# KLab/YAIK

Hardware: AMD Instinct MI355X
Metric: Mpix/s tile encode (alpha reject + 7 gradient passes + 8x8 range quant), 8K RGBA (higher is better)
Workload: dtype u8/int32 (+f32 mode-selection sums)

## Files before the change

### yaik_amd/csrc/yk_api.hip

```cpp
#include "yk_common.h"
#ifdef YK_TEST_HOOKS
#include "../../include/yaik_hip_test.h"
#endif
#include <cstdio>
#include <cstring>
#include <utility>
#include <vector>

int yk_fail(yk_ctx* c, int code, const char* what, hipError_t e) {
    if (c && c->err.empty()) {
        c->err = what ? what : "error";
        if (e != hipSuccess) { c->err += ": "; c->err += hipGetErrorString(e); }
    }
    return code;
}

int yk_refuse(yk_ctx* c, int code, const char* what) {
    if (c) c->err = what ? what : "error";
    return code;
}

static void yk_input_changed(yk_ctx* c) {
    c->encoded = false; c->alphaDone = false; c->alphaFinished = false; c->avBatchValid = false; c->mipValid = false; c->img.sb.valid = false; c->pal.valid = false;
    c->cornersReady = false; c->ppActive = false; c->ppLastBit = 0; c->previewFresh = false;
// ... 26 lines not shown
    YK_HIP(c, M.alphaUnitBox.alloc(s, yk_alpha_units(c->fullW, c->mtH) * F * 4, 16));
    static const int sh[7][2] = { {4,4},{4,3},{3,4},{3,3},{3,2},{2,3},{2,2} };
    size_t cur = 0, oBm[7], oBm0b, oCov, oInfo, oRun;
    auto place = [&](size_t bytesPerFrame) { const size_t o = cur; cur = up(cur + bytesPerFrame * F + 16, 256); return o; };
    for (int i = 0; i < 7; i++) {
        const int bx = (sh[i][0] == 2) ? 32 : 64, by = (sh[i][1] == 2) ? 32 : 64;
        const size_t bits = (size_t)((c->fullW + bx - 1) / bx) * ((c->h + by - 1) / by) * ((bx >> sh[i][0]) * (by >> sh[i][1]));
        c->bitmapBytes[i] = bits >> 3;
        fs.bitmap[i] = up(c->bitmapBytes[i] + 4, 16);
        oBm[i] = place(fs.bitmap[i]);
    }
    const size_t nB64 = (size_t)((c->fullW + 63) / 64) * ((c->h + 63) / 64);
    fs.bm0b = up(nB64 * 4, 16); oBm0b = place(fs.bm0b);
    fs.coverage = up(MT, 8); oCov = place(fs.coverage * sizeof(uint16_t));
    fs.tileInfo = up(T8, 2); oInfo = place(fs.tileInfo * sizeof(uint2));
    fs.runSums = up((T8 + 7) / 8, 4); oRun = place(fs.runSums * sizeof(uint32_t));
    if (cur >= ((size_t)1 << 32)) return yk_fail(c, YK_ERR_BAD_ARG, "image too large for 32-bit offsets into the small-output arena");
    YK_HIP(c, M.small.alloc(s, cur));
    YK_HIP(c, hipMemset(M.small, 0, cur));
    B.small = M.small;
    for (int i = 0; i < 7; i++) B.bitmap[i] = B.small + oBm[i];
    B.bm0b = B.small + oBm0b; B.coverage = reinterpret_cast<uint16_t*>(B.small + oCov);
    B.tileInfo = reinterpret_cast<uint2*>(B.small + oInfo); B.runSums = reinterpret_cast<uint32_t*>(B.small + oRun);
    fs.tileDef = 3 * T8; fs.tileCount = 3 * T8; fs.slots = 3 * T8 * YK_SLOT;
    YK_HIP(c, M.tileDef.alloc(s, fs.tileDef * F, 16));
    YK_HIP(c, M.tileCount.alloc(s, fs.tileCount * F, 16));
    YK_HIP(c, M.slots.alloc(s, fs.slots * F, 16));
    c->nScanBlocks = (int)((T8 + 1023) / 1024);
    fs.blockN = (size_t)c->nScanBlocks * 2;
    YK_HIP(c, M.blockSums.alloc(s, fs.blockN * F));
    YK_HIP(c, M.blockCnt.alloc(s, fs.blockN * F));
    YK_HIP(c, hipMemset(M.blockCnt, 0, fs.blockN * F * sizeof(uint32_t)));
    YK_HIP(c, M.totals.alloc(s, 8 * F));
    fs.defsOut = 3 * T8;
    YK_HIP(c, M.defsOut.alloc(s, fs.defsOut * F, 16));
    c->nibStride = T8 * YK_SLOT + 64;
    fs.nibOut = 3 * c->nibStride;
    YK_HIP(c, M.nibOut.alloc(s, fs.nibOut * F, 16));
    B.keep = M.keep; B.bounds = M.bounds; B.tileDef = M.tileDef; B.tileCount = M.tileCount; B.slots = M.slots;
    B.blockSums = M.blockSums; B.blockCnt = M.blockCnt; B.totals = M.totals; B.defsOut = M.defsOut; B.nibOut = M.nibOut;
    c->dstValid = false;
    return YK_OK;
}
static int yk_alloc_image(yk_ctx* c) {
    const int rc = yk_alloc_image_run(c);
    if (rc) yk_free_image(c);
// ... 759 lines not shown
```

### yaik_amd/csrc/yk_common.h

```cpp
#pragma once
#include <hip/hip_runtime.h>
#include <stdint.h>
#include <stddef.h>
#include <memory>
#include <string>
#include <vector>
#include "../../include/yaik_hip.h"

#define YK_BLK      64
#define YK_LSTRIDE  68
#define YK_LROWS    65
#define YK_EV_RING  64
#define YK_SLOT     32
#define YK_NUM_STAGES 11
#define YK_STAGE_RING 16

struct YkFrameStrides {
    unsigned long long plane, keep, bitmap[7], coverage, tileDef, tileCount, slots, blockN, defsOut, nibOut;
    unsigned long long bm0b, tileInfo, runSums;
};

enum { YK_EVSET_ALPHA = 1, YK_EVSET_PACK = 2 };
enum { YK_EV_A0, YK_EV_E0, YK_EV_E1, YK_EV_P1, YK_EV_N };
struct YkEvRing {
    hipEvent_t ev[YK_EV_RING][YK_EV_N] = {};
    YkEvRing() = default;
    YkEvRing(const YkEvRing&) = delete; YkEvRing& operator=(const YkEvRing&) = delete;
    ~YkEvRing() { for (auto& set : ev) for (hipEvent_t e : set) if (e) (void)hipEventDestroy(e); }
};

// ... 23 lines not shown
    int w, h;
    int hAvail;
    int y0;
    int fullH;
    int rejectFactor, startMode, wantDst;
    int ablate;
    const uint8_t* keep;
    const int32_t* bounds;
    uint8_t* bitmap[7];
    uint16_t* coverage;
    uint16_t* tileDef;
    uint8_t*  tileCount;
    uint8_t*  slots;
    uint32_t* blockCnt;
    int32_t*  dst[3];
    int tilesW, tilesH, mtW, mtH;
    int xBB64, yBB64, xBB32, yBB32;
    int nFrames;
    const uint8_t* qtab;
    uint8_t* small;
    uint32_t oBm[7], oBm0b, oCov, oInfo, oRun;
    uint4* pixCache;
    YkFrameStrides fs;
};

#define YK_SB_COUNTS 9
struct YkStreamRec { uint8_t* rgb[7]; uint8_t* pix; uint8_t* type; };
struct YkStreamsBatch {
    YkBuf<uint32_t> owner;
    YkBuf<uint32_t> cScratch;
    YkBuf<uint32_t> r1Scratch;
    YkBuf<uint32_t> counts;
    YkBuf<uint8_t> out;
    YkBuf<YkStreamRec> tab;
    std::vector<yk_frame_streams> table; bool valid = false;
    int what = 0;
};

struct YkPalette {
    YkBuf<uint8_t> scratch;
    YkBuf<uint8_t> out;
    YkBuf<uint32_t> carry;
    bool carryFresh = true;
    std::vector<uint8_t> segHost;
    std::vector<uint32_t> lenBase;
    int nSeg = 0; bool valid = false;
};

struct YkPaletteDec {
    YkBuf<uint8_t> scratch;
    YkBuf<uint8_t> out;
    YkBuf<uint8_t> stage;
    std::vector<size_t> slotOff, slotLen;
    std::vector<uint32_t> statusHost;
    size_t statusOff = 0;
    int nSeg = 0; bool valid = false;
};

#ifndef YK_ALPHA_R
#define YK_ALPHA_R 4
#endif
static inline size_t yk_alpha_units(int fullW, int mtH) { return (size_t)((fullW / 4 + 63) / 64) * (size_t)((mtH + YK_ALPHA_R - 1) / YK_ALPHA_R); }

struct YkImageBufs {
    YkBuf<uint8_t> keep; YkBuf<int32_t> bounds;
    YkBuf<int> alphaUnitBox;
    YkBuf<uint8_t> small;
    YkBuf<uint16_t> tileDef; YkBuf<uint8_t> tileCount, slots;
    YkBuf<int32_t> dst[3];
    YkBuf<uint32_t> blockSums, blockCnt, totals;
    YkBuf<unsigned long long> exportSizes;
    YkBuf<uint16_t> defsOut; YkBuf<uint8_t> nibOut;
    YkBuf<uint32_t> latticeOwner; YkBuf<uint8_t> cornerStream; YkBuf<uint32_t> cornerScratch;
    YkBuf<uint32_t> cornerEdgeIdx;
    YkBuf<uint16_t> covCh;
    YkBuf<uint8_t> mapped3;
    YkBuf<uint32_t> ppBitmap; YkBuf<uint8_t> ppStream; YkBuf<uint32_t> ppScratch;
    YkBuf<int32_t> preview;
    YkBuf<uint8_t> r1Slots, r1Params; YkBuf<uint32_t> r1Cnt; YkBuf<uint8_t> r1Pix, r1Type;
    YkBuf<uint4> pixCache;
    YkStreamsBatch sb;
};

struct yk_ctx {
    int device = -1;
    int numCU = 256;
    const uint8_t* qtab = nullptr;
    hipStream_t ownStream = nullptr;
    hipStream_t stream = nullptr;
    std::string err;
    int fullW = 0, fullH = 0, nPlanes = 0, y0 = 0, h = 0, halo = 0;
    int tilesW = 0, tilesH = 0, mtW = 0, mtH = 0;
    int nFrames = 1, curFrame = 0;
    YkFrameStrides fs = {};
    struct Bases {
        const int32_t* plane[4];
        uint8_t* keep;
        int32_t* bounds;
        uint8_t* bitmap[7]; uint16_t* coverage; uint16_t* tileDef; uint8_t* tileCount; uint8_t* slots;
        uint32_t* blockSums;
        uint32_t* blockCnt;
        uint32_t* totals;
        uint16_t* defsOut;
        uint8_t* nibOut;
        uint8_t* small;
        uint8_t* bm0b; uint2* tileInfo; uint32_t* runSums;
    } B = {};
    int strideElems = 0;
    YkBuf<int32_t> ownedPlanes;
    YkBuf<uint8_t> pxStage;
    hipEvent_t evPixCopy = nullptr;
    int boundsOff = 8;
    bool alphaDone = false, alphaFinished = false;
    int32_t hostBounds[4] = {0, 0, 0, 0}; int hostDiscard = 1, hostHasChunk = 0;
    size_t bitmapBytes[7] = {};
    int32_t dstFill = -1; bool dstValid = false;
    hipEvent_t evHandoff = nullptr;
// ... 128 lines not shown
```

### yaik_amd/csrc/yk_encode2.hip

```cpp
#include "yk_common.h"
#include "yk_curves.h"
#include "yk_device.h"
#include <mutex>

__constant__ float c_curve2[6][16] = YK_CURVE_TABLE;

#define LS YK_LSTRIDE
#ifdef YK_TEST_HOOKS
#define YK2_ABLATE(bit) ((P.ablate & (bit)) != 0)
#else
#define YK2_ABLATE(bit) false
#endif

__device__ __forceinline__ int y2_byte(uint32_t w, int ch) { return (w >> (8 * ch)) & 255; }
__device__ __forceinline__ uint32_t y2_absdiff(uint32_t a, uint32_t b) { uint32_t r; asm("v_sad_u32 %0, %1, %2, 0" : "=v"(r) : "v"(a), "v"(b)); return r; }
__device__ __forceinline__ int y2_round6(int v) { return (v & ~3) | (v >> 6); }
__device__ __forceinline__ int y2_round6p(int v) { v = min(v + 1, 255); return (v & ~3) | (v >> 6); }

typedef short y2s2 __attribute__((ext_vector_type(2)));
typedef unsigned short y2u2 __attribute__((ext_vector_type(2)));
__device__ __forceinline__ y2u2 y2_u2(uint32_t w) { return __builtin_bit_cast(y2u2, w); }
__device__ __forceinline__ y2s2 y2_s2(y2u2 v) { return __builtin_bit_cast(y2s2, v); }
__device__ __forceinline__ y2u2 y2_splat(int v) { const unsigned short t = (unsigned short)v; return (y2u2){ t, t }; }
__device__ __forceinline__ y2s2 y2_splats(int v) { const short t = (short)v; return (y2s2){ t, t }; }
// ... 454 lines not shown
        int L[16];
        for (int i = 0; i < cnt; i++) {
            L[i] = __float2int_rz(__fadd_rn((float)BN, __fmul_rn(c_curve2[m][i], (float)R)));
            if (L[i] != BN + __float2int_rz(__fmul_rn(c_curve2[m][i], (float)R))) bad++;
        }
        for (int v = mn; v <= mx; v++) {
            int best = 1 << 30, bi = 0;
            for (int n = 0; n < cnt; n++) { const int dd = abs(L[n] - v); if (dd < best) { best = dd; bi = n; } }
            const uint4 row = tab[(size_t)(R - YK2_QR0) * YK2_QROWS + (v - BN + 2)];
            const uint32_t w = m < 2 ? row.x : (m < 4 ? row.y : row.z);
            const uint32_t hb = (m & 1) ? (w >> 16) : (w & 0xFFFFu);
            const int ix = (row.w >> (4 * m)) & 15;
            if (hb != y2_f16_bits(best) || ix != bi) bad++;
        }
    }
    if (bad) atomicAdd(mismatches, bad);
}

#define YK2_RUN 16
template <int K> __device__ __forceinline__ uint32_t y2_writelane_k(uint32_t v, uint32_t old) { asm("v_writelane_b32 %0, %1, %2" : "+v"(old) : "s"(v), "n"(K)); return old; }
__device__ __forceinline__ uint32_t y2_writelane(uint32_t v, int k, uint32_t old) {
    switch (k) {
        case 0: return y2_writelane_k<0>(v, old); case 1: return y2_writelane_k<1>(v, old); case 2: return y2_writelane_k<2>(v, old);
        case 3: return y2_writelane_k<3>(v, old); case 4: return y2_writelane_k<4>(v, old); default: return y2_writelane_k<5>(v, old);
    }
}
#ifdef YK2_TIMING
__device__ unsigned long long g_y2_times[65536 * 16];
#define YK2_PROBE(i) do { if ((i) == 0 && lane == 0 && unit < 65536) { g_y2_times[(size_t)unit * 16 + 10] = 0; g_y2_times[(size_t)unit * 16 + 11] = 0; g_y2_times[(size_t)unit * 16 + 12] = y2_t_entry; g_y2_times[(size_t)unit * 16 + 13] = ((unsigned long long)y2_xcc << 32) | y2_hwid; } if (lane == 0 && unit < 65536) { g_y2_times[(size_t)unit * 16 + 2 * (i)] = __builtin_amdgcn_s_memtime(); g_y2_times[(size_t)unit * 16 + 2 * (i) + 1] = __builtin_amdgcn_s_memrealtime(); } } while (0)
extern "C" int yk_debug_wave_times(unsigned long long* out) { return (int)hipMemcpyFromSymbol(out, HIP_SYMBOL(g_y2_times), sizeof(g_y2_times)); }
#else
#define YK2_PROBE(i) do { } while (0)
#endif
#define YK2_LUTW 84
#ifndef YK2_WIN
#define YK2_WIN 16
#endif
#ifndef YK2_PREF
#define YK2_PREF 8
#endif
#ifndef YK2_RVWIN
#define YK2_RVWIN 8
#endif

#define Y2_QUAD_X 0xB1
#define Y2_QUAD_Y 0x4E
template <int CTRL> __device__ __forceinline__ int y2_quad(int v) { return __builtin_amdgcn_update_dpp(v, v, CTRL, 0xF, 0xF, true); }
// ... 30 lines not shown
}

template <bool WANT_DST, bool MODE3>
__global__ __launch_bounds__(64, 4) void yk_encode2_kernel(const YkEncodeParams P) {
    constexpr int kStart = MODE3 ? 3 : 0;
    constexpr int kPixWords = 17 * LS, kLutWords = WANT_DST ? 16 * YK2_LUTW : 0;
    __shared__ __attribute__((aligned(16))) uint32_t s_mem[kPixWords > kLutWords ? kPixWords : kLutWords];
    uint32_t* const s_pix = s_mem;
    uint32_t (*const s_lut)[YK2_LUTW] = reinterpret_cast<uint32_t (*)[YK2_LUTW]>(s_mem);
    __shared__ uint32_t s_bm[24];
    __shared__ uint8_t s_list[64];
    __shared__ __attribute__((aligned(16))) float s_curve[WANT_DST ? 6 : 1][16];
    __shared__ __attribute__((aligned(16))) float s_rcp[256];
    __shared__ __attribute__((aligned(16))) uint32_t s_aux[432];
    uint32_t* const s_lat = s_aux;
    float (*const s_chain)[68] = reinterpret_cast<float (*)[68]>(s_aux);
    float* const s_err = reinterpret_cast<float*>(s_aux + 408);
    __shared__ uint32_t s_range[3 * 64];
    __shared__ __attribute__((aligned(16))) uint32_t s_sp[3 * 4 * 8 + 3 * 4 * 16];

    uint32_t* const s_tile = s_aux + 416;
    __shared__ uint32_t s_iwTest[WANT_DST ? 1024 : 1];
    uint32_t* const s_iw = WANT_DST ? s_iwTest : s_mem;
    static_assert(WANT_DST || kPixWords >= 1024, "index words need 4 KB");

    const int lane = threadIdx.x;
    __builtin_amdgcn_s_setprio(3);
#ifdef YK2_TIMING
    const unsigned long long y2_t_entry = __builtin_amdgcn_s_memrealtime();
    const unsigned y2_hwid = __builtin_amdgcn_s_getreg((4 << 0) | (0 << 6) | (31 << 11)), y2_xcc = __builtin_amdgcn_s_getreg((20 << 0) | (0 << 6) | (31 << 11));
#endif
    typedef const __attribute__((address_space(4))) YkEncodeParams* Y2ParamPtr;
    auto strip = [&](const int slot, const int xcd, const int lane, Y2ParamPtr const Pp) {
    const __attribute__((address_space(4))) YkEncodeParams& P = *Pp;
    const int nBf = P.xBB64 * P.yBB64, nB = nBf * P.nFrames;
    const int grp = slot / (YK2_RUN * 4);
    const int unit = (grp * 8 + ((xcd + grp) & 7)) * (YK2_RUN * 4) + (slot - grp * (YK2_RUN * 4));
    int L = unit >> 2; const int wave = unit & 3;
    if (L >= nB) return;
    size_t fr = 0;
    if (P.nFrames > 1) { fr = (size_t)(L / nBf); L -= (int)fr * nBf; }
    const int32_t* const pl0 = P.plane[0] + fr * P.fs.plane; const int32_t* const pl1 = P.plane[1] + fr * P.fs.plane; const int32_t* const pl2 = P.plane[2] + fr * P.fs.plane;
    const uint8_t* const keepP = P.keep ? P.keep + fr * P.fs.keep : nullptr;
    const int32_t* const boundsP = P.bounds ? P.bounds + fr * 16 : nullptr;
    uint8_t* const slotsP = P.slots + fr * P.fs.slots;
    uint32_t* const blockCntP = P.blockCnt + fr * P.fs.blockN;
    const int BY = L / P.xBB64, BX = L - BY * P.xBB64;
    const int w = P.w, h = P.h;

    YK2_PROBE(0);
    if (lane < 24) s_bm[lane] = 0;
    {
        const int g4 = (lane & 15) * 4, r0 = lane >> 4;
        const int gx = BX * 64 + g4;
        const bool inX = gx + 3 < w;
        const int gxc = min(gx, w - 4);
        const int gyS = BY * 64 + wave * 16;
        const int gyB = min(gyS, P.hAvail - 1);
        const size_t rowBase = (size_t)gyB * (size_t)P.strideElems;
        const char* const b0 = reinterpret_cast<const char*>(pl0 + rowBase);
        const char* const b1 = reinterpret_cast<const char*>(pl1 + rowBase);
        const char* const b2 = reinterpret_cast<const char*>(pl2 + rowBase);
        int4 R[4], G[4], B[4];
#pragma unroll
        for (int k = 0; k < 4; k++) {
            const int rel = min(gyS + r0 + 4 * k, P.hAvail - 1) - gyB;
            const uint32_t off = (uint32_t)(rel * P.strideElems + gxc) * 4u;
            R[k] = *reinterpret_cast<const int4*>(b0 + off);
            G[k] = *reinterpret_cast<const int4*>(b1 + off);
            B[k] = *reinterpret_cast<const int4*>(b2 + off);
        }
        int4 Rb, Gb, Bb;
        {
            const int rel = min(gyS + 16, P.hAvail - 1) - gyB;
            const uint32_t off = (uint32_t)(rel * P.strideElems + gxc) * 4u;
            Rb = *reinterpret_cast<const int4*>(b0 + off);
            Gb = *reinterpret_cast<const int4*>(b1 + off);
            Bb = *reinterpret_cast<const int4*>(b2 + off);
        }
        uint32_t hcol;
        const int hr = min(max(lane - 32, 0), 16);
        {
            const int rel = min(gyS + hr, P.hAvail - 1) - gyB;
            const uint32_t off = (uint32_t)(rel * P.strideElems + min(BX * 64 + 64, w - 1)) * 4u;
            hcol = y2_pack3(*reinterpret_cast<const int32_t*>(b0 + off), *reinterpret_cast<const int32_t*>(b1 + off), *reinterpret_cast<const int32_t*>(b2 + off));
        }
        const float4 rc4 = *reinterpret_cast<const float4*>(P.qtab + YK2_QBYTES + (size_t)lane * 16);

        __builtin_amdgcn_s_setprio(0);
        uint4 o[4], ob;
#pragma unroll
        for (int k = 0; k < 4; k++) {
            o[k] = make_uint4(y2_pack3(R[k].x, G[k].x, B[k].x), y2_pack3(R[k].y, G[k].y, B[k].y), y2_pack3(R[k].z, G[k].z, B[k].z), y2_pack3(R[k].w, G[k].w, B[k].w));
            *reinterpret_cast<uint4*>(&s_pix[(r0 + 4 * k) * LS + g4]) = o[k];
        }
        ob = make_uint4(y2_pack3(Rb.x, Gb.x, Bb.x), y2_pack3(Rb.y, Gb.y, Bb.y), y2_pack3(Rb.z, Gb.z, Bb.z), y2_pack3(Rb.w, Gb.w, Bb.w));
        if (lane < 16) *reinterpret_cast<uint4*>(&s_pix[16 * LS + g4]) = ob;
        if (BX * 64 + 64 > w) {
            if (!inX) {
#pragma unroll
                for (int k = 0; k < 4; k++) *reinterpret_cast<uint4*>(&s_pix[(r0 + 4 * k) * LS + g4]) = make_uint4(o[k].w, o[k].w, o[k].w, o[k].w);
                if (lane < 16) *reinterpret_cast<uint4*>(&s_pix[16 * LS + g4]) = make_uint4(ob.w, ob.w, ob.w, ob.w);
            }
        }
        if (lane >= 32 && lane <= 48) s_pix[hr * LS + 64] = hcol;
        *reinterpret_cast<float4*>(&s_rcp[lane * 4]) = rc4;

    }
    __syncthreads();
    YK2_PROBE(1);

    const int q = lane >> 4, cx = y2_cell_x(lane & 15), cy = y2_cell_y(lane & 15);
    const int bxCell = q * 16 + cx * 4, byCell = wave * 16 + cy * 4;
    const int gxCell = BX * 64 + bxCell, gyCell = BY * 64 + byCell;
    const int lcell = (cy * 4) * LS + bxCell;
    const int lat = cy * 17 + q * 4 + cx;
    const bool mtIn = (BX * 64 + q * 16 < w) && (BY * 64 + wave * 16 < h);

    uint32_t pw[16];
#pragma unroll
    for (int r = 0; r < 4; r++) {
        const uint4 t = *reinterpret_cast<const uint4*>(&s_pix[lcell + r * LS]);
        pw[r * 4 + 0] = t.x; pw[r * 4 + 1] = t.y; pw[r * 4 + 2] = t.z; pw[r * 4 + 3] = t.w;
    }

    unsigned long long cov = 0ULL;
    unsigned long long evaluated = 0ULL;
    {
        bool dead = !mtIn;
        {
            const int lim = 4 * P.rejectFactor + 1;
// ... 28 lines not shown
            y2s2 rg[16], bb[8];
#pragma unroll
            for (int k = 0; k < 16; k++) rg[k] = y2_rg(pw[k]);
#pragma unroll
            for (int k = 0; k < 8; k++) bb[k] = y2_bb(pw[2 * k], pw[2 * k + 1]);
            const Y2Pass S = { s_lat, lat, cx, cy, rg, bb, deadLanes, stripInside, gxCell, gyCell, w, h, P.rejectFactor, s_bm, bxCell, byCell, s_pix, s_list, s_range, lane };
            if (deadLanes == 0ULL) y2_grad_pass<4, 4, true>(S, cov, evaluated);
            else y2_grad_pass<4, 4>(S, cov, evaluated);
            if (~(cov | deadLanes) != 0ULL) {
                y2_grad_pass<4, 3>(S, cov, evaluated);
                y2_grad_pass<3, 4>(S, cov, evaluated);
                y2_grad_pass<3, 3>(S, cov, evaluated);
                y2_grad_pass<3, 2>(S, cov, evaluated);
                y2_grad_pass<2, 3>(S, cov, evaluated);
                y2_grad_pass<2, 2>(S, cov, evaluated);
            }
#pragma unroll
            for (int r = 0; r < 4; r++) {
                const uint4 t = *reinterpret_cast<const uint4*>(&s_pix[lcell + r * LS]);
                pw[r * 4 + 0] = t.x; pw[r * 4 + 1] = t.y; pw[r * 4 + 2] = t.z; pw[r * 4 + 3] = t.w;
            }
        }
    }
    const int mtIdx = ((BY * 64 + wave * 16) >> 4) * P.mtW + ((BX * 64 + q * 16) >> 4);
    __syncthreads();
    YK2_PROBE(2);
    uint8_t* const small = P.small;
    const uint32_t bmv = s_bm[lane < 24 ? lane : 0];
    auto bmWord = [&](const int k) -> uint32_t { return (uint32_t)__builtin_amdgcn_readlane((int)bmv, k); };
    const uint32_t i64 = (uint32_t)(BY * P.xBB64 + BX);
    const uint32_t frU = (uint32_t)fr;
    uint32_t off32 = ~0u, val32 = 0u;
    {
        const uint32_t w1 = (uint32_t)wave & 1u, w2 = (uint32_t)wave >> 1;
        uint32_t off8 = 0u, val8 = 0u;
        off8 = y2_writelane(P.oBm0b + frU * (uint32_t)P.fs.bm0b + i64 * 4u + (uint32_t)wave, 0, off8);
        val8 = y2_writelane((bmWord(0) >> (4 * wave)) & 0xFu, 0, val8);
        off8 = y2_writelane(P.oBm[1] + frU * (uint32_t)P.fs.bitmap[1] + i64 * 4u + (uint32_t)wave, 1, off8);
        val8 = y2_writelane(bmWord(1) >> (8 * wave), 1, val8);
        off8 = y2_writelane(P.oBm[2] + frU * (uint32_t)P.fs.bitmap[2] + i64 * 4u + (uint32_t)wave, 2, off8);
        val8 = y2_writelane(bmWord(2) >> (8 * wave), 2, val8);
        if (lane < 3) *(small + off8) = (uint8_t)val8;
        const unsigned long long t = ((cov >> 2) ^ cov) & 0x0C0C0C0C0C0C0C0CULL;
        const unsigned long long covRM = cov ^ t ^ (t << 2);
        uint32_t off16 = ((lane & 15) == 0 && mtIn) ? P.oCov + (frU * (uint32_t)P.fs.coverage + (uint32_t)mtIdx) * 2u : ~0u;
        uint32_t val16 = (uint32_t)((covRM >> (q * 16)) & 0xFFFFULL);
        off16 = y2_writelane(P.oBm[3] + frU * (uint32_t)P.fs.bitmap[3] + (i64 * 4u + (uint32_t)wave) * 2u, 1, off16);
        val16 = y2_writelane(bmWord(3 + (int)w2) >> (16 * w1), 1, val16);
#pragma unroll
        for (int sx = 0; sx < 2; sx++) {
            const bool in = BX * 2 + sx < P.xBB32;
            off16 = y2_writelane(in ? P.oBm[5] + frU * (uint32_t)P.fs.bitmap[5] + ((uint32_t)((BY * P.xBB32 + BX * 2 + sx) * 4 + wave)) * 2u : ~0u, 2 + sx, off16);
            val16 = y2_writelane(bmWord(9 + sx * 2 + (int)w2) >> (16 * w1), 2 + sx, val16);
        }
        if (off16 != ~0u) *reinterpret_cast<uint16_t*>(small + off16) = (uint16_t)val16;
        if (P.pixCache != nullptr) {
            const bool cellIn = (gxCell < w) && (gyCell < h);
            if (cellIn && !((cov >> lane) & 1ULL)) {
                const uint32_t strip = (uint32_t)((BY * 4 + wave) * P.xBB64 + BX);
                uint4* dstp = P.pixCache + (size_t)strip * 256 + lane;
#pragma unroll
                for (int r = 0; r < 4; r++) dstp[r * 64] = make_uint4(pw[r * 4 + 0], pw[r * 4 + 1], pw[r * 4 + 2], pw[r * 4 + 3]);
            }
        }
        {
            const bool in = BY * 2 + (int)w2 < P.yBB32;
            off32 = y2_writelane(in ? P.oBm[4] + frU * (uint32_t)P.fs.bitmap[4] + ((uint32_t)(((BY * 2 + (int)w2) * P.xBB64 + BX) * 2) + w1) * 4u : ~0u, 1, off32);
            val32 = y2_writelane(bmWord(5 + (int)w2 * 2 + (int)w1), 1, val32);
#pragma unroll
            for (int sx = 0; sx < 2; sx++) {
                const bool in6 = in && (BX * 2 + sx < P.xBB32);
                off32 = y2_writelane(in6 ? P.oBm[6] + frU * (uint32_t)P.fs.bitmap[6] + ((uint32_t)(((BY * 2 + (int)w2) * P.xBB32 + BX * 2 + sx) * 2) + w1) * 4u : ~0u, 2 + sx, off32);
                val32 = y2_writelane(bmWord(13 + ((int)w2 * 2 + sx) * 2 + (int)w1), 2 + sx, val32);
            }
        }
    }
    YK2_PROBE(3);
    int cxB = 0, cyB = 0, cw = w, chh = P.fullH, discard = 1;
    if (boundsP) {
        const int b0 = boundsP[0], b1 = boundsP[1], b2 = boundsP[2], b3 = boundsP[3];
        discard = (b0 == 0 && b1 == 0 && b2 == w && b3 == P.fullH) ? 1 : 0;
        cxB = (b0 >> 3) << 3; cyB = (b1 >> 3) << 3;
        cw = (((b2 + 7) >> 3) << 3) - cxB; chh = (((b3 + 7) >> 3) << 3) - cyB;
    }
    const int cxl = cx & 1, cyl = cy & 1;
    const int tgx = gxCell - cxl * 4, tgyl = gyCell - cyl * 4, tgy = tgyl + P.y0;
    const bool tileIn = (tgx + 8 <= w) && (tgyl + 8 <= h);
    const bool part = tileIn && tgx >= cxB && tgx < cxB + cw && tgy >= cyB && tgy < cyB + chh && (tgx + 8 <= cw) && (tgy + 8 <= chh);
    const bool keepMT = (keepP == nullptr) || discard || (mtIn && keepP[mtIdx] != 0);
    const bool tileLive = part && keepMT;
    const int l00 = lane & ~3;
    const uint32_t quadN = (uint32_t)((~cov) >> l00) & 15u;
    const int v00 = (int)(quadN & 1u), v01 = (int)((quadN >> 2) & 1u);
    const bool valid = tileLive && ((quadN >> (lane & 3)) & 1u);
    const int nTop = __popc(quadN & 3u), nBot = __popc(quadN >> 2);
    const int tileIdx = (tgyl >> 3) * P.tilesW + (tgx >> 3);
    const size_t T8 = (size_t)P.tilesW * P.tilesH;
    const int tw = lane >> 2;
    const bool writer = ((lane & 3) == 0) && tileIn;
    const unsigned long long validMask = __ballot(valid);
    const bool fullTiles = !WANT_DST && __ballot(tileLive && quadN != 15u && quadN != 0u) == 0ULL;

    {
        const int n16 = (tileLive && !YK2_ABLATE(1)) ? (nTop + nBot) : 0;
        if ((P.tilesW & 7) == 0) {
#pragma unroll
            for (int r = 0; r < 2; r++) {
                const bool mine = writer && ((cy >> 1) == r);
                const unsigned long long b0 = __ballot(mine && (n16 & 1)), b1 = __ballot(mine && (n16 & 2)), b2 = __ballot(mine && (n16 & 4));
                const unsigned long long bd = __ballot(mine && n16 > 0);
                const int row = ((BY * 64 + wave * 16) >> 3) + r;
                off32 = y2_writelane(row < P.tilesH ? P.oRun + (frU * (uint32_t)P.fs.runSums + (uint32_t)(row * (P.tilesW >> 3) + BX)) * 4u : ~0u, 4 + r, off32);
                val32 = y2_writelane((uint32_t)(__popcll(b0) + 2 * __popcll(b1) + 4 * __popcll(b2)) | ((uint32_t)__popcll(bd) << 16), 4 + r, val32);
            }
        } else if (writer && n16 > 0) {
            atomicAdd(&blockCntP[((size_t)tileIdx >> 10) * 2], 16u * (uint32_t)n16);
            atomicAdd(&blockCntP[((size_t)tileIdx >> 10) * 2 + 1], 1u);
        }
        if (off32 != ~0u) *reinterpret_cast<uint32_t*>(small + off32) = val32;
    }

    YK2_STAT(70, validMask != 0ULL ? 1 : 0); YK2_STAT(74, __popcll(validMask));
    { const int nv = __popcll(validMask); YK2_STAT(120 + (nv == 0 ? 0 : nv <= 4 ? 1 : nv <= 8 ? 2 : nv <= 16 ? 3 : nv <= 32 ? 4 : nv < 64 ? 5 : 6), 1); (void)nv; }
    uint32_t defs01 = 0u, defs2c = 0u;
    if (validMask != 0ULL && !YK2_ABLATE(1)) {
        uint32_t* lut = &s_lut[WANT_DST ? tw : 0][0];
        if (WANT_DST) {
            s_curve[lane >> 4][lane & 15] = c_curve2[lane >> 4][lane & 15];
            if (lane < 32) s_curve[4 + (lane >> 4)][lane & 15] = c_curve2[4 + (lane >> 4)][lane & 15];
        }
        const int j4 = lane & 3;
        const int nValidLanes = __popcll(validMask);
        const bool spread = nValidLanes <= 4 && !WANT_DST;
        const int vRank = (int)__builtin_amdgcn_mbcnt_hi((uint32_t)(validMask >> 32), __builtin_amdgcn_mbcnt_lo((uint32_t)validMask, 0u));
        uint32_t slotOff[4];
#pragma unroll
        for (int r = 0; r < 4; r++) {
            const int yIn = cyl * 4 + r;
            const int pos = (yIn < 4) ? (yIn * 4 * nTop + (cxl ? 4 * v00 : 0))
                                      : (16 * nTop + (yIn - 4) * 4 * nBot + (cxl ? 4 * v01 : 0));
            slotOff[r] = (uint32_t)tileIdx * (uint32_t)YK_SLOT + (uint32_t)(pos >> 1);
        }
        int tmn[3], tmx[3];
        {
            y2u2 mnRB = y2_splat(0xFFFF), mxRB = y2_splat(0), mnG = y2_splat(0xFFFF), mxG = y2_splat(0);
            if (valid) {
#pragma unroll
                for (int k = 0; k < 16; k += 2) {
// ... 331 lines not shown
        hipLaunchKernelGGL(yk_qtab_kernel, dim3(YK2_QNR), dim3(320), 0, c->stream, reinterpret_cast<uint4*>(t));
        {
            float rcp[256]; rcp[0] = 0.0f;
            for (int v = 1; v < 256; v++) rcp[v] = 1.0f / (float)v;
            YK_HIP(c, hipMemcpyAsync(t + YK2_QBYTES, rcp, sizeof rcp, hipMemcpyHostToDevice, c->stream));
        }
        hipLaunchKernelGGL(yk_deftab_kernel, dim3(225), dim3(YK2_DEFN1), 0, c->stream, reinterpret_cast<uint32_t*>(t + YK2_QBYTES + YK2_RCPBYTES));
        YK_HIP(c, hipGetLastError());
        YK_HIP(c, hipStreamSynchronize(c->stream));
        g_qtab[c->device] = t;
    }
    c->qtab = g_qtab[c->device];
    return YK_OK;
}
void yk_selftest_qtab_launch(yk_ctx* c, int* mismatches) {
    hipLaunchKernelGGL(yk_selftest_qtab_kernel, dim3(256), dim3(256), 0, c->stream, reinterpret_cast<const uint4*>(c->qtab),
                       reinterpret_cast<const uint32_t*>(c->qtab + YK2_QBYTES + YK2_RCPBYTES), mismatches);
}

int yk_launch_encode2(yk_ctx* c, const YkEncodeParams& P) {
    if (!P.qtab) return yk_fail(c, YK_ERR_STATE, "quantiser table missing");
    if (P.startMode != 0 && P.startMode != 3) return yk_fail(c, YK_ERR_BAD_ARG, "startMode must be 0 or 3");
    const int nB = P.xBB64 * P.yBB64 * P.nFrames, group = 8 * YK2_RUN;
    dim3 grid(((nB + group - 1) / group) * group * 4);
    if (P.wantDst) {
        if (P.startMode) hipLaunchKernelGGL((yk_encode2_kernel<true, true>), grid, dim3(64), 0, c->stream, P);
        else hipLaunchKernelGGL((yk_encode2_kernel<true, false>), grid, dim3(64), 0, c->stream, P);
    } else {
        if (P.startMode) hipLaunchKernelGGL((yk_encode2_kernel<false, true>), grid, dim3(64), 0, c->stream, P);
        else hipLaunchKernelGGL((yk_encode2_kernel<false, false>), grid, dim3(64), 0, c->stream, P);
    }
    YK_HIP(c, hipGetLastError());
    return YK_OK;
}
```

### yaik_amd/csrc/yk_stages.hip

```cpp
#include "yk_common.h"
#ifdef YK_TEST_HOOKS
#include "../../include/yaik_hip_test.h"
#endif
#include "yk_device.h"

typedef int yk_i4 __attribute__((ext_vector_type(4)));
#ifndef YK_ALPHA_WAVES
#define YK_ALPHA_WAVES 3
#endif
__global__ __launch_bounds__(64 * YK_ALPHA_WAVES, 4) void yk_alpha_kernel(const int32_t* __restrict__ alpha0, int strideElems, int w, int h, int y0,
                                                      uint8_t* __restrict__ keep0, int mtW, int mtH, unsigned long long planeStride,
                                                      unsigned long long keepStride, yk_i4* __restrict__ unitBox0, unsigned total) {
    const int lane = threadIdx.x & 63;
    const int vecPerRow = w >> 2;
    const int nSeg = (vecPerRow + 63) >> 6;
    const int nUnits = nSeg * ((mtH + YK_ALPHA_R - 1) / YK_ALPHA_R);
    const unsigned uu = blockIdx.x * YK_ALPHA_WAVES + (threadIdx.x >> 6);
    if (uu >= total) return;
    const int f = (int)(uu / (unsigned)nUnits), u = (int)(uu - (unsigned)f * (unsigned)nUnits);
    const int32_t* alpha = alpha0 + (size_t)f * planeStride;
    uint8_t* keep = keep0 + (size_t)f * keepStride;
    const int tyU = u / nSeg, seg = u - tyU * nSeg, ty0 = tyU * YK_ALPHA_R;
    const int xv = seg * 64 + lane;
    const bool inX = xv < vecPerRow;
// ... 269 lines not shown
    return YK_OK;
}

int yk_launch_encode(yk_ctx* c, int rejectFactor, int mode3BitOnly, int wantDst, bool batch) {
    const YkFrameView V = yk_frame(c, batch ? 0 : c->curFrame);
    YkEncodeParams P;
    for (int i = 0; i < 4; i++) P.plane[i] = V.plane[i];
    P.strideElems = c->strideElems; P.w = c->fullW; P.h = c->h; P.hAvail = c->h + c->halo; P.y0 = c->y0; P.fullH = c->fullH;
    P.rejectFactor = rejectFactor; P.startMode = mode3BitOnly ? 3 : 0; P.wantDst = wantDst; P.ablate = c->ablate;
    P.keep = (c->nPlanes == 4) ? V.keep : nullptr;
    P.bounds = (c->nPlanes == 4) ? V.bounds + c->boundsOff : nullptr;
    for (int i = 0; i < 7; i++) P.bitmap[i] = V.bitmap[i];
    P.coverage = V.coverage; P.tileDef = V.tileDef; P.tileCount = V.tileCount; P.slots = V.slots;
    P.blockCnt = c->kernelVersion == 2 ? V.blockCnt : nullptr;
    for (int i = 0; i < 3; i++) P.dst[i] = c->img.dst[i];
    P.tilesW = c->tilesW; P.tilesH = c->tilesH; P.mtW = c->mtW; P.mtH = c->mtH;
    P.xBB64 = (c->fullW + 63) / 64; P.yBB64 = (c->h + 63) / 64; P.xBB32 = (c->fullW + 31) / 32; P.yBB32 = (c->h + 31) / 32;
    P.nFrames = batch ? c->nFrames : 1; P.fs = c->fs;
    P.qtab = c->qtab;
    P.small = V.small;
    auto off = [&](const void* p) { return (uint32_t)(static_cast<const uint8_t*>(p) - V.small); };
    for (int i = 0; i < 7; i++) P.oBm[i] = off(V.bitmap[i]);
    P.oBm0b = off(V.bm0b); P.oCov = off(V.coverage); P.oInfo = off(V.tileInfo); P.oRun = off(V.runSums);
    P.pixCache = nullptr; c->pixCacheValid = false;
    if (c->pixCacheOn && !batch && c->kernelVersion == 2 && c->nFrames == 1) {
        if (!c->img.pixCache) YK_HIP(c, c->img.pixCache.alloc(c->stream, (size_t)P.xBB64 * 64 * ((size_t)(c->h + 15) / 16 * 16) / 4, 4096));
        P.pixCache = c->img.pixCache; c->pixCacheValid = true;
    }
    if (c->kernelVersion == 2) return yk_launch_encode2(c, P);
    if (batch) return yk_fail(c, YK_ERR_STATE, "batches need kernel version 2");
    if (c->nPlanes == 4) {
        hipLaunchKernelGGL(yk_alpha_publish_kernel, dim3(1), dim3(1), 0, c->stream, V.bounds, c->boundsOff, c->fullW, c->fullH);
        P.bounds = V.bounds;
    }
    if (!g_crossCheckLauncher) return yk_fail(c, YK_ERR_STATE, "kernel version 1 is not part of this library: register it with yk_set_cross_check_launcher");
    if (g_crossCheckLauncher(c->stream, &P) != 0) return yk_fail(c, YK_ERR_HIP, "cross-check kernel launch", hipGetLastError());
    return YK_OK;
}

int yk_launch_pack(yk_ctx* c, bool batch) {
    const size_t T8 = (size_t)c->tilesW * c->tilesH;
    const int nb = c->nScanBlocks, F = batch ? c->nFrames : 1;
    const YkFrameView V = yk_frame(c, batch ? 0 : c->curFrame);
    if (c->kernelVersion != 2) hipLaunchKernelGGL(yk_scan1_kernel, dim3(nb), dim3(1024), 0, c->stream, V.tileCount, T8, V.blockCnt);
    const bool v2 = c->kernelVersion == 2;
    const uint32_t* runSums = (v2 && (c->tilesW & 7) == 0) ? V.runSums : nullptr;
// ... 78 lines not shown
```

Measured before the change: 235,800.

## Table-drive bitmap output offsets, hoist keep/bounds scalar loads, use magic division

Precomputes a per-wave, per-lane output geometry table on the host so the kernel's small-arena bitmap and run-sum writes become a single table lookup, replacing chains of writelane and address arithmetic. Keep and bounds are fetched early with scalar loads that overlap with the pixel loads. Integer divisions by the block width and frame size become multiply-shift magic division. Spare waves no longer exit before the early loads, and a host verification tool for the divider is added. This adds a table allocation and a limit on block count per launch, and relies on inline asm and on the table staying in sync with the layout.

```diff
diff --git a/yaik_amd/csrc/yk_api.hip b/yaik_amd/csrc/yk_api.hip
--- a/yaik_amd/csrc/yk_api.hip
+++ b/yaik_amd/csrc/yk_api.hip
@@ -72,6 +72,17 @@
     for (int i = 0; i < 7; i++) B.bitmap[i] = B.small + oBm[i];
     B.bm0b = B.small + oBm0b; B.coverage = reinterpret_cast<uint16_t*>(B.small + oCov);
     B.tileInfo = reinterpret_cast<uint2*>(B.small + oInfo); B.runSums = reinterpret_cast<uint32_t*>(B.small + oRun);
+    {
+        YkOutGeom g;
+        for (int i = 0; i < 7; i++) g.oBm[i] = (uint32_t)oBm[i];
+        g.oBm0b = (uint32_t)oBm0b; g.oRun = (uint32_t)oRun;
+        g.xBB64 = (c->fullW + 63) / 64; g.xBB32 = (c->fullW + 31) / 32; g.yBB32 = (c->h + 31) / 32; g.tilesW = c->tilesW; g.tilesH = c->tilesH;
+        YkOutRow tab[4][YK2_OT_ROWS];
+        yk_out_table_fill(tab, g, fs);
+        YK_HIP(c, M.outTab.alloc(s, sizeof tab / sizeof(uint4)));
+        YK_HIP(c, hipMemcpy(M.outTab, tab, sizeof tab, hipMemcpyHostToDevice));
+        c->divXBB64 = yk_udiv_make((uint32_t)g.xBB64); c->divNBf = yk_udiv_make((uint32_t)nB64);
+    }
     fs.tileDef = 3 * T8; fs.tileCount = 3 * T8; fs.slots = 3 * T8 * YK_SLOT;
     YK_HIP(c, M.tileDef.alloc(s, fs.tileDef * F, 16));
     YK_HIP(c, M.tileCount.alloc(s, fs.tileCount * F, 16));
diff --git a/yaik_amd/csrc/yk_common.h b/yaik_amd/csrc/yk_common.h
--- a/yaik_amd/csrc/yk_common.h
+++ b/yaik_amd/csrc/yk_common.h
@@ -6,6 +6,7 @@
 #include <string>
 #include <vector>
 #include "../../include/yaik_hip.h"
+#include "yk_udiv.h"
 
 #define YK_BLK      64
 #define YK_LSTRIDE  68
@@ -75,7 +76,42 @@
     uint32_t oBm[7], oBm0b, oCov, oInfo, oRun;
     uint4* pixCache;
     YkFrameStrides fs;
-};
+    YkUdiv divXBB64, divNBf;
+    const uint4* outTab;
+    uint32_t outFrame0;
+};
+
+#define YK2_OT_ROWS 16
+#define YK2_OT_NONE 0xFFFFFFFFu
+struct YkOutRow { uint32_t base, sF, sX, sY, limX, limY, sel, pad; };
+static_assert(sizeof(YkOutRow) == 32, "two 16-byte loads per row");
+struct YkOutGeom { uint32_t oBm[7], oBm0b, oRun; int xBB64, xBB32, yBB32, tilesW, tilesH; };
+inline void yk_out_table_fill(YkOutRow (*T)[YK2_OT_ROWS], const YkOutGeom& g, const YkFrameStrides& fs) {
+    const uint32_t none = YK2_OT_NONE;
+    auto lim = [](int n, int step) -> uint32_t { return n <= 0 ? 0u : (uint32_t)((n + step - 1) / step); };
+    for (int wv = 0; wv < 4; wv++) {
+        const uint32_t w1 = (uint32_t)wv & 1u, w2 = (uint32_t)wv >> 1, X64 = (uint32_t)g.xBB64, X32 = (uint32_t)g.xBB32;
+        YkOutRow* R = T[wv];
+        for (int k = 0; k < YK2_OT_ROWS; k++) R[k] = YkOutRow{ 0u, 0u, 0u, 0u, 0u, 0u, 0u, 0u };
+        auto sel = [](uint32_t idx, uint32_t sh, uint32_t bits) { return idx | (sh << 8) | ((32u - bits) << 16); };
+        R[1] = YkOutRow{ g.oBm0b + wv, (uint32_t)fs.bm0b, 4u, 4u * X64, none, none, sel(0, 4u * wv, 4), 0u };
+        R[2] = YkOutRow{ g.oBm[1] + wv, (uint32_t)fs.bitmap[1], 4u, 4u * X64, none, none, sel(1, 8u * wv, 32), 0u };
+        R[3] = YkOutRow{ g.oBm[2] + wv, (uint32_t)fs.bitmap[2], 4u, 4u * X64, none, none, sel(2, 8u * wv, 32), 0u };
+        R[4] = YkOutRow{ g.oBm[3] + 2u * wv, (uint32_t)fs.bitmap[3], 8u, 8u * X64, none, none, sel(3 + w2, 16u * w1, 32), 0u };
+        for (uint32_t sx = 0; sx < 2; sx++)
+            R[5 + sx] = YkOutRow{ g.oBm[5] + (sx * 4u + wv) * 2u, (uint32_t)fs.bitmap[5], 16u, 8u * X32, lim(g.xBB32 - (int)sx, 2), none, sel(9 + sx * 2 + w2, 16u * w1, 32), 0u };
+        const uint32_t limY32 = lim(g.yBB32 - (int)w2, 2);
+        R[8] = YkOutRow{ g.oBm[4] + w2 * 8u * X64 + w1 * 4u, (uint32_t)fs.bitmap[4], 8u, 16u * X64, none, limY32, sel(5 + w2 * 2 + w1, 0, 32), 0u };
+        for (uint32_t sx = 0; sx < 2; sx++)
+            R[9 + sx] = YkOutRow{ g.oBm[6] + w2 * 8u * X32 + sx * 8u + w1 * 4u, (uint32_t)fs.bitmap[6], 16u, 16u * X32, lim(g.xBB32 - (int)sx, 2), limY32,
+                                  sel(13 + (w2 * 2 + sx) * 2 + w1, 0, 32), 0u };
+        if ((g.tilesW & 7) == 0) {
+            const uint32_t runsW = (uint32_t)(g.tilesW >> 3);
+            for (int r = 0; r < 2; r++)
+                R[11 + r] = YkOutRow{ g.oRun + (uint32_t)(wv * 2 + r) * runsW * 4u, (uint32_t)fs.runSums * 4u, 4u, 32u * runsW, none, lim(g.tilesH - wv * 2 - r, 8), 0u, 0u };
+        }
+    }
+}
 
 #define YK_SB_COUNTS 9
 struct YkStreamRec { uint8_t* rgb[7]; uint8_t* pix; uint8_t* type; };
@@ -119,6 +155,7 @@
     YkBuf<uint8_t> keep; YkBuf<int32_t> bounds;
     YkBuf<int> alphaUnitBox;
     YkBuf<uint8_t> small;
+    YkBuf<uint4> outTab;
     YkBuf<uint16_t> tileDef; YkBuf<uint8_t> tileCount, slots;
     YkBuf<int32_t> dst[3];
     YkBuf<uint32_t> blockSums, blockCnt, totals;
@@ -146,6 +183,7 @@
     int tilesW = 0, tilesH = 0, mtW = 0, mtH = 0;
     int nFrames = 1, curFrame = 0;
     YkFrameStrides fs = {};
+    YkUdiv divXBB64 = {}, divNBf = {};
     struct Bases {
         const int32_t* plane[4];
         uint8_t* keep;
diff --git a/yaik_amd/csrc/yk_encode2.hip b/yaik_amd/csrc/yk_encode2.hip
--- a/yaik_amd/csrc/yk_encode2.hip
+++ b/yaik_amd/csrc/yk_encode2.hip
@@ -500,7 +500,8 @@
 __device__ __forceinline__ uint32_t y2_writelane(uint32_t v, int k, uint32_t old) {
     switch (k) {
         case 0: return y2_writelane_k<0>(v, old); case 1: return y2_writelane_k<1>(v, old); case 2: return y2_writelane_k<2>(v, old);
-        case 3: return y2_writelane_k<3>(v, old); case 4: return y2_writelane_k<4>(v, old); default: return y2_writelane_k<5>(v, old);
+        case 3: return y2_writelane_k<3>(v, old); case 4: return y2_writelane_k<4>(v, old); case 5: return y2_writelane_k<5>(v, old);
+        case 11: return y2_writelane_k<11>(v, old); default: return y2_writelane_k<12>(v, old);
     }
 }
 #ifdef YK2_TIMING
@@ -577,6 +578,7 @@
     uint32_t* const s_tile = s_aux + 416;
     __shared__ uint32_t s_iwTest[WANT_DST ? 1024 : 1];
     uint32_t* const s_iw = WANT_DST ? s_iwTest : s_mem;
+    uint32_t* const s_park = WANT_DST ? s_iwTest : s_sp;
     static_assert(WANT_DST || kPixWords >= 1024, "index words need 4 KB");
 
     const int lane = threadIdx.x;
@@ -592,19 +594,21 @@
     const int grp = slot / (YK2_RUN * 4);
     const int unit = (grp * 8 + ((xcd + grp) & 7)) * (YK2_RUN * 4) + (slot - grp * (YK2_RUN * 4));
     int L = unit >> 2; const int wave = unit & 3;
-    if (L >= nB) return;
-    size_t fr = 0;
-    if (P.nFrames > 1) { fr = (size_t)(L / nBf); L -= (int)fr * nBf; }
+    const bool spare = L >= nB;
+    L = spare ? 0 : L;
+    const uint32_t frU = yk_udiv((uint32_t)L, P.divNBf.mul, P.divNBf.shift);
+    L -= (int)frU * nBf;
+    const size_t fr = frU;
     const int32_t* const pl0 = P.plane[0] + fr * P.fs.plane; const int32_t* const pl1 = P.plane[1] + fr * P.fs.plane; const int32_t* const pl2 = P.plane[2] + fr * P.fs.plane;
-    const uint8_t* const keepP = P.keep ? P.keep + fr * P.fs.keep : nullptr;
-    const int32_t* const boundsP = P.bounds ? P.bounds + fr * 16 : nullptr;
-    uint8_t* const slotsP = P.slots + fr * P.fs.slots;
-    uint32_t* const blockCntP = P.blockCnt + fr * P.fs.blockN;
-    const int BY = L / P.xBB64, BX = L - BY * P.xBB64;
+    const int BY = (int)yk_udiv((uint32_t)L, P.divXBB64.mul, P.divXBB64.shift), BX = L - BY * P.xBB64;
     const int w = P.w, h = P.h;
+    const int mt0 = (BY * 4 + wave) * P.mtW + BX * 4;
 
     YK2_PROBE(0);
     if (lane < 24) s_bm[lane] = 0;
+    typedef uint32_t y2_u32x2 __attribute__((ext_vector_type(2)));
+    typedef int32_t y2_i32x4 __attribute__((ext_vector_type(4)));
+    y2_u32x2 keep8; y2_i32x4 bnd;
     {
         const int g4 = (lane & 15) * 4, r0 = lane >> 4;
         const int gx = BX * 64 + g4;
@@ -641,8 +645,25 @@
             hcol = y2_pack3(*reinterpret_cast<const int32_t*>(b0 + off), *reinterpret_cast<const int32_t*>(b1 + off), *reinterpret_cast<const int32_t*>(b2 + off));
         }
         const float4 rc4 = *reinterpret_cast<const float4*>(P.qtab + YK2_QBYTES + (size_t)lane * 16);
+        const uint4* const orow = P.outTab + (wave * YK2_OT_ROWS + (lane & (YK2_OT_ROWS - 1))) * 2;
+        const uint4 ta = orow[0], tb = orow[1];
+        {
+            const bool rowIn = BY * 64 + wave * 16 < h;
+            const uintptr_t args = reinterpret_cast<uintptr_t>(Pp);
+            const uintptr_t kpIn = reinterpret_cast<uintptr_t>(P.keep) + fr * P.fs.keep + (uintptr_t)(mt0 & ~3);
+            const uintptr_t bpIn = reinterpret_cast<uintptr_t>(P.bounds) + fr * 64;
+            const uintptr_t kp = (P.keep != nullptr && rowIn) ? kpIn : args, bp = P.bounds != nullptr ? bpIn : args;
+            asm volatile("s_load_dwordx2 %0, %2, 0x0\n\ts_load_dwordx4 %1, %3, 0x0" : "=&s"(keep8), "=&s"(bnd) : "s"(kp), "s"(bp));
+        }
 
         __builtin_amdgcn_s_setprio(0);
+        if (spare) return;
+        {
+            const uint32_t frT = frU + P.outFrame0;
+            const uint32_t o = ta.x + frT * ta.y + (uint32_t)BX * ta.z + (uint32_t)BY * ta.w;
+            s_park[lane] = ((uint32_t)BX < tb.x && (uint32_t)BY < tb.y) ? o : YK2_OT_NONE;
+            s_park[64 + lane] = tb.z;
+        }
         uint4 o[4], ob;
 #pragma unroll
         for (int k = 0; k < 4; k++) {
@@ -662,6 +683,7 @@
         *reinterpret_cast<float4*>(&s_rcp[lane * 4]) = rc4;
 
     }
+    asm volatile("s_waitcnt lgkmcnt(0)" : "+s"(keep8), "+s"(bnd));
     __syncthreads();
     YK2_PROBE(1);
 
@@ -736,37 +758,21 @@
             }
         }
     }
-    const int mtIdx = ((BY * 64 + wave * 16) >> 4) * P.mtW + ((BX * 64 + q * 16) >> 4);
+    const int mtIdx = mt0 + q;
     __syncthreads();
     YK2_PROBE(2);
     uint8_t* const small = P.small;
-    const uint32_t bmv = s_bm[lane < 24 ? lane : 0];
-    auto bmWord = [&](const int k) -> uint32_t { return (uint32_t)__builtin_amdgcn_readlane((int)bmv, k); };
-    const uint32_t i64 = (uint32_t)(BY * P.xBB64 + BX);
-    const uint32_t frU = (uint32_t)fr;
-    uint32_t off32 = ~0u, val32 = 0u;
+    const uint32_t tabOff = s_park[lane], tabSel = s_park[64 + lane];
+    const uint32_t tabVal = (s_bm[tabSel & 31u] >> ((tabSel >> 8) & 31u)) & (~0u >> (tabSel >> 16));
+    uint32_t off32 = (uint32_t)lane - 8u < 5u ? tabOff : ~0u;
+    uint32_t val32 = (uint32_t)lane - 8u < 3u ? tabVal : 0u;
     {
-        const uint32_t w1 = (uint32_t)wave & 1u, w2 = (uint32_t)wave >> 1;
-        uint32_t off8 = 0u, val8 = 0u;
-        off8 = y2_writelane(P.oBm0b + frU * (uint32_t)P.fs.bm0b + i64 * 4u + (uint32_t)wave, 0, off8);
-        val8 = y2_writelane((bmWord(0) >> (4 * wave)) & 0xFu, 0, val8);
-        off8 = y2_writelane(P.oBm[1] + frU * (uint32_t)P.fs.bitmap[1] + i64 * 4u + (uint32_t)wave, 1, off8);
-        val8 = y2_writelane(bmWord(1) >> (8 * wave), 1, val8);
-        off8 = y2_writelane(P.oBm[2] + frU * (uint32_t)P.fs.bitmap[2] + i64 * 4u + (uint32_t)wave, 2, off8);
-        val8 = y2_writelane(bmWord(2) >> (8 * wave), 2, val8);
-        if (lane < 3) *(small + off8) = (uint8_t)val8;
+        if ((uint32_t)lane - 1u < 3u) *(small + tabOff) = (uint8_t)tabVal;
         const unsigned long long t = ((cov >> 2) ^ cov) & 0x0C0C0C0C0C0C0C0CULL;
         const unsigned long long covRM = cov ^ t ^ (t << 2);
         uint32_t off16 = ((lane & 15) == 0 && mtIn) ? P.oCov + (frU * (uint32_t)P.fs.coverage + (uint32_t)mtIdx) * 2u : ~0u;
         uint32_t val16 = (uint32_t)((covRM >> (q * 16)) & 0xFFFFULL);
-        off16 = y2_writelane(P.oBm[3] + frU * (uint32_t)P.fs.bitmap[3] + (i64 * 4u + (uint32_t)wave) * 2u, 1, off16);
-        val16 = y2_writelane(bmWord(3 + (int)w2) >> (16 * w1), 1, val16);
-#pragma unroll
-        for (int sx = 0; sx < 2; sx++) {
-            const bool in = BX * 2 + sx < P.xBB32;
-            off16 = y2_writelane(in ? P.oBm[5] + frU * (uint32_t)P.fs.bitmap[5] + ((uint32_t)((BY * P.xBB32 + BX * 2 + sx) * 4 + wave)) * 2u : ~0u, 2 + sx, off16);
-            val16 = y2_writelane(bmWord(9 + sx * 2 + (int)w2) >> (16 * w1), 2 + sx, val16);
-        }
+        if ((uint32_t)lane - 4u < 3u) { off16 = tabOff; val16 = tabVal; }
         if (off16 != ~0u) *reinterpret_cast<uint16_t*>(small + off16) = (uint16_t)val16;
         if (P.pixCache != nullptr) {
             const bool cellIn = (gxCell < w) && (gyCell < h);
@@ -777,22 +783,11 @@
                 for (int r = 0; r < 4; r++) dstp[r * 64] = make_uint4(pw[r * 4 + 0], pw[r * 4 + 1], pw[r * 4 + 2], pw[r * 4 + 3]);
             }
         }
-        {
-            const bool in = BY * 2 + (int)w2 < P.yBB32;
-            off32 = y2_writelane(in ? P.oBm[4] + frU * (uint32_t)P.fs.bitmap[4] + ((uint32_t)(((BY * 2 + (int)w2) * P.xBB64 + BX) * 2) + w1) * 4u : ~0u, 1, off32);
-            val32 = y2_writelane(bmWord(5 + (int)w2 * 2 + (int)w1), 1, val32);
-#pragma unroll
-            for (int sx = 0; sx < 2; sx++) {
-                const bool in6 = in && (BX * 2 + sx < P.xBB32);
-                off32 = y2_writelane(in6 ? P.oBm[6] + frU * (uint32_t)P.fs.bitmap[6] + ((uint32_t)(((BY * 2 + (int)w2) * P.xBB32 + BX * 2 + sx) * 2) + w1) * 4u : ~0u, 2 + sx, off32);
-                val32 = y2_writelane(bmWord(13 + ((int)w2 * 2 + sx) * 2 + (int)w1), 2 + sx, val32);
-            }
-        }
     }
     YK2_PROBE(3);
     int cxB = 0, cyB = 0, cw = w, chh = P.fullH, discard = 1;
-    if (boundsP) {
-        const int b0 = boundsP[0], b1 = boundsP[1], b2 = boundsP[2], b3 = boundsP[3];
+    if (P.bounds != nullptr) {
+        const int b0 = bnd.x, b1 = bnd.y, b2 = bnd.z, b3 = bnd.w;
         discard = (b0 == 0 && b1 == 0 && b2 == w && b3 == P.fullH) ? 1 : 0;
         cxB = (b0 >> 3) << 3; cyB = (b1 >> 3) << 3;
         cw = (((b2 + 7) >> 3) << 3) - cxB; chh = (((b3 + 7) >> 3) << 3) - cyB;
@@ -801,7 +796,8 @@
     const int tgx = gxCell - cxl * 4, tgyl = gyCell - cyl * 4, tgy = tgyl + P.y0;
     const bool tileIn = (tgx + 8 <= w) && (tgyl + 8 <= h);
     const bool part = tileIn && tgx >= cxB && tgx < cxB + cw && tgy >= cyB && tgy < cyB + chh && (tgx + 8 <= cw) && (tgy + 8 <= chh);
-    const bool keepMT = (keepP == nullptr) || discard || (mtIn && keepP[mtIdx] != 0);
+    const uint32_t keep4 = (uint32_t)((((unsigned long long)keep8.y << 32) | keep8.x) >> (8 * (mt0 & 3)));
+    const bool keepMT = (P.keep == nullptr) || discard || (mtIn && ((keep4 >> (8 * q)) & 0xFFu) != 0u);
     const bool tileLive = part && keepMT;
     const int l00 = lane & ~3;
     const uint32_t quadN = (uint32_t)((~cov) >> l00) & 15u;
@@ -818,16 +814,17 @@
     {
         const int n16 = (tileLive && !YK2_ABLATE(1)) ? (nTop + nBot) : 0;
         if ((P.tilesW & 7) == 0) {
-#pragma unroll
-            for (int r = 0; r < 2; r++) {
-                const bool mine = writer && ((cy >> 1) == r);
-                const unsigned long long b0 = __ballot(mine && (n16 & 1)), b1 = __ballot(mine && (n16 & 2)), b2 = __ballot(mine && (n16 & 4));
-                const unsigned long long bd = __ballot(mine && n16 > 0);
-                const int row = ((BY * 64 + wave * 16) >> 3) + r;
-                off32 = y2_writelane(row < P.tilesH ? P.oRun + (frU * (uint32_t)P.fs.runSums + (uint32_t)(row * (P.tilesW >> 3) + BX)) * 4u : ~0u, 4 + r, off32);
-                val32 = y2_writelane((uint32_t)(__popcll(b0) + 2 * __popcll(b1) + 4 * __popcll(b2)) | ((uint32_t)__popcll(bd) << 16), 4 + r, val32);
+            if (validMask != 0ULL) {
+#pragma unroll
+                for (int r = 0; r < 2; r++) {
+                    const bool mine = writer && ((cy >> 1) == r);
+                    const unsigned long long b0 = __ballot(mine && (n16 & 1)), b1 = __ballot(mine && (n16 & 2)), b2 = __ballot(mine && (n16 & 4));
+                    const unsigned long long bd = __ballot(mine && n16 > 0);
+                    val32 = y2_writelane((uint32_t)(__popcll(b0) + 2 * __popcll(b1) + 4 * __popcll(b2)) | ((uint32_t)__popcll(bd) << 16), 11 + r, val32);
+                }
             }
         } else if (writer && n16 > 0) {
+            uint32_t* const blockCntP = P.blockCnt + fr * P.fs.blockN;
             atomicAdd(&blockCntP[((size_t)tileIdx >> 10) * 2], 16u * (uint32_t)n16);
             atomicAdd(&blockCntP[((size_t)tileIdx >> 10) * 2 + 1], 1u);
         }
@@ -838,6 +835,7 @@
     { const int nv = __popcll(validMask); YK2_STAT(120 + (nv == 0 ? 0 : nv <= 4 ? 1 : nv <= 8 ? 2 : nv <= 16 ? 3 : nv <= 32 ? 4 : nv < 64 ? 5 : 6), 1); (void)nv; }
     uint32_t defs01 = 0u, defs2c = 0u;
     if (validMask != 0ULL && !YK2_ABLATE(1)) {
+        uint8_t* const slotsP = P.slots + fr * P.fs.slots;
         uint32_t* lut = &s_lut[WANT_DST ? tw : 0][0];
         if (WANT_DST) {
             s_curve[lane >> 4][lane & 15] = c_curve2[lane >> 4][lane & 15];
@@ -1215,6 +1213,8 @@
     if (!P.qtab) return yk_fail(c, YK_ERR_STATE, "quantiser table missing");
     if (P.startMode != 0 && P.startMode != 3) return yk_fail(c, YK_ERR_BAD_ARG, "startMode must be 0 or 3");
     const int nB = P.xBB64 * P.yBB64 * P.nFrames, group = 8 * YK2_RUN;
+    if ((long long)P.xBB64 * P.yBB64 * P.nFrames + group > (long long)YK_UDIV_LIMIT) return yk_fail(c, YK_ERR_BAD_ARG, "too many blocks for one launch");
+    if (!P.outTab) return yk_fail(c, YK_ERR_STATE, "output table missing");
     dim3 grid(((nB + group - 1) / group) * group * 4);
     if (P.wantDst) {
         if (P.startMode) hipLaunchKernelGGL((yk_encode2_kernel<true, true>), grid, dim3(64), 0, c->stream, P);
diff --git a/yaik_amd/csrc/yk_stages.hip b/yaik_amd/csrc/yk_stages.hip
--- a/yaik_amd/csrc/yk_stages.hip
+++ b/yaik_amd/csrc/yk_stages.hip
@@ -315,6 +315,8 @@
     auto off = [&](const void* p) { return (uint32_t)(static_cast<const uint8_t*>(p) - V.small); };
     for (int i = 0; i < 7; i++) P.oBm[i] = off(V.bitmap[i]);
     P.oBm0b = off(V.bm0b); P.oCov = off(V.coverage); P.oInfo = off(V.tileInfo); P.oRun = off(V.runSums);
+    P.divXBB64 = c->divXBB64; P.divNBf = c->divNBf;
+    P.outTab = c->img.outTab; P.outFrame0 = batch ? 0u : (uint32_t)c->curFrame;
     P.pixCache = nullptr; c->pixCacheValid = false;
     if (c->pixCacheOn && !batch && c->kernelVersion == 2 && c->nFrames == 1) {
         if (!c->img.pixCache) YK_HIP(c, c->img.pixCache.alloc(c->stream, (size_t)P.xBB64 * 64 * ((size_t)(c->h + 15) / 16 * 16) / 4, 4096));
diff --git a/yaik_amd/csrc/yk_udiv.h b/yaik_amd/csrc/yk_udiv.h
--- /dev/null
+++ b/yaik_amd/csrc/yk_udiv.h
@@ -0,0 +1,25 @@
+#pragma once
+#include <cstdint>
+
+#define YK_UDIV_LIMIT (1u << 29)
+
+struct YkUdiv { uint32_t mul, shift; };
+
+inline YkUdiv yk_udiv_make(uint32_t d) {
+    YkUdiv r = { 0u, 0u };
+    if (d == 0) return r;
+    while ((d >> r.shift) > 1u) r.shift++;
+    r.mul = (uint32_t)((((uint64_t)1 << (31 + r.shift)) + d - 1) / d);
+    return r;
+}
+
+#if defined(__HIPCC__)
+__host__ __device__
+#endif
+inline uint32_t yk_udiv(uint32_t n, uint32_t mul, uint32_t shift) {
+#if defined(__HIP_DEVICE_COMPILE__)
+    return __umulhi(2u * n + 1u, mul) >> shift;
+#else
+    return (uint32_t)(((uint64_t)(2u * n + 1u) * mul) >> 32) >> shift;
+#endif
+}
diff --git a/yaik_amd/host/udiv_tool.cpp b/yaik_amd/host/udiv_tool.cpp
--- /dev/null
+++ b/yaik_amd/host/udiv_tool.cpp
@@ -0,0 +1,49 @@
+#include <cinttypes>
+#include <cstdio>
+#include <cstdlib>
+#include <cstring>
+#include "../csrc/yk_udiv.h"
+
+static uint64_t checked = 0, bad = 0, firstD = 0, firstN = 0;
+static inline void check(uint32_t n, uint32_t d, const YkUdiv& r) {
+    checked++;
+    if (yk_udiv(n, r.mul, r.shift) != n / d) { if (!bad) { firstD = d; firstN = n; } bad++; }
+}
+
+int main(int argc, char** argv) {
+    if (argc < 4) { fprintf(stderr, "usage: udiv_tool all <dMax> <factor> | ranges <dMax> <seed> <nRand>\n"); return 2; }
+    const uint32_t dMax = (uint32_t)strtoul(argv[2], nullptr, 10);
+    uint64_t maxN = 0;
+    if (!strcmp(argv[1], "all")) {
+        const uint64_t factor = strtoull(argv[3], nullptr, 10);
+        for (uint32_t d = 1; d <= dMax; d++) {
+            const YkUdiv r = yk_udiv_make(d);
+            const uint64_t end = (uint64_t)d * factor;
+            if (end > YK_UDIV_LIMIT) { fprintf(stderr, "d * factor beyond the limit\n"); return 2; }
+            for (uint32_t n = 0; n < (uint32_t)end; n++) check(n, d, r);
+            if (end - 1 > maxN) maxN = end - 1;
+        }
+    } else if (!strcmp(argv[1], "ranges") && argc >= 5) {
+        uint64_t rng = strtoull(argv[3], nullptr, 10) * 0x9E3779B97F4A7C15ull + 1;
+        const int nRand = atoi(argv[4]);
+        const uint64_t lim = YK_UDIV_LIMIT;
+        for (uint32_t d = 1; d <= dMax; d++) {
+            const YkUdiv r = yk_udiv_make(d);
+            const uint64_t ks[7] = { 1, 2, 3, 1023, 1024, 1025, (lim - 1) / d };
+            for (uint64_t k : ks) {
+                const uint64_t a = k * d;
+                if (a - 1 < lim) check((uint32_t)(a - 1), d, r);
+                if (a < lim) check((uint32_t)a, d, r);
+            }
+            check(0u, d, r); check(1u, d, r); check((uint32_t)(lim - 1), d, r); check((uint32_t)(lim - 2), d, r);
+            for (int i = 0; i < nRand; i++) {
+                rng ^= rng << 13; rng ^= rng >> 7; rng ^= rng << 17;
+                check((uint32_t)(rng % lim), d, r);
+            }
+        }
+        maxN = lim - 1;
+    } else { fprintf(stderr, "unknown mode\n"); return 2; }
+    printf("{\"mode\": \"%s\", \"dMax\": %u, \"limit\": %u, \"maxNumerator\": %" PRIu64 ", \"checked\": %" PRIu64 ", \"mismatches\": %" PRIu64
+           ", \"firstBad\": [%" PRIu64 ", %" PRIu64 "]}\n", argv[1], dMax, (unsigned)YK_UDIV_LIMIT, maxN, checked, bad, firstD, firstN);
+    return bad ? 1 : 0;
+}
```

Result: faster. 240,600, median of 6 (+2.0%).
